# talmolab/sleap-nn

Measured on AMD Instinct MI355X. Metric: frames/sec bottom-up UNet 1024x1024 inference, higher is better.
Workload: dtype f32

## Files before the change

### sleap_nn_amd/csrc/w16_kernels.hip

```cpp
#include <type_traits>

#include "common.h"
#include "net_kernels.h"

namespace ph {

typedef float f32x4 __attribute__((ext_vector_type(4)));

constexpr int V_TW = 16, V_TH = 32;
constexpr int V_HH = V_TH + 2;
constexpr int V_PLANE_E = V_HH * 9;
constexpr int V_PLANE_PIECES = (V_PLANE_E + 15) / 16;
constexpr int V_PLANE_FLOATS = V_PLANE_PIECES * 256;
constexpr int V_HALO_FLOATS = 2 * V_PLANE_FLOATS;
constexpr int v_w_floats(int nb) { return 16 * nb * 256; }

__global__ __launch_bounds__(256) void w16_pack_kernel(const float* __restrict__ src, float* __restrict__ dst, int chunks, int nbs) {
  const int per = v_w_floats(nbs), total = chunks * per;
  for (int i = blockIdx.x * 256 + threadIdx.x; i < total; i += gridDim.x * 256) {
    const int chunk = i / per, r = i - chunk * per;
    const int e = r & 3, n = (r >> 2) & 15, kq = (r >> 6) & 3, nb = (r >> 8) % nbs, pos = (r >> 8) / nbs;
    const int xi = pos >> 2, nu = pos & 3;
    const int row = nb * 16 + n, kc = 4 * kq + e;
    const float* w = src + ((size_t)chunk * 9 * 32 + row) * 16 + kc;
    const int ts = 32 * 16;
    float h[3];
#pragma unroll
    for (int kx = 0; kx < 3; ++kx) {
      const float g0 = w[(0 * 3 + kx) * ts], g1 = w[(1 * 3 + kx) * ts], g2 = w[(2 * 3 + kx) * ts];
      h[kx] = xi == 0 ? g0 : (xi == 1 ? 0.5f * ((g0 + g2) + g1) : (xi == 2 ? 0.5f * ((g0 + g2) - g1) : g2));
    }
    dst[i] = nu == 0 ? h[0] : (nu == 1 ? 0.5f * ((h[0] + h[2]) + h[1]) : (nu == 2 ? 0.5f * ((h[0] + h[2]) - h[1]) : h[2]));
  }
}
int64_t w16_pack_floats(int chunks, int nbs) { return (int64_t)chunks * v_w_floats(nbs); }
int launch_w16_pack(const float* wpack, float* w16, int chunks, int nbs, hipStream_t s) {
  PH_REQUIRE(nbs == 1 || nbs == 2, "w16 pack: one or two N blocks of 16 channels");
  hipLaunchKernelGGL(w16_pack_kernel, dim3(std::min(chunks * v_w_floats(nbs) / 256, 256)), dim3(256), 0, s, wpack, w16, chunks, nbs);
  PH_HIP_CHECK(hipGetLastError());
  return PH_OK;
}

template <int CHUNKS, int NB, bool TWO = false, bool HEAD = false>
__global__ __launch_bounds__(512, 2) void conv3x3_w16_kernel(ConvArgs a) {
  constexpr int V_W_FLOATS = v_w_floats(NB);
  extern __shared__ __attribute__((aligned(16))) float lds[];
  float* const wl = lds;
  float* const hbuf = lds + CHUNKS * V_W_FLOATS;
  const int tid = threadIdx.x;
  const int lane = tid & 63;
  const int wave = __builtin_amdgcn_readfirstlane(tid >> 6);
  const int li = lane & 15, kq = lane >> 4;
  float m1 = -1.f;
  asm volatile("" : "+v"(m1));
  const int tiles_x = (a.W + V_TW - 1) / V_TW;
  const int tiles_y = (a.H + V_TH - 1) / V_TH;
  const int total = tiles_x * tiles_y * a.B;

  const __amdgpu_buffer_rsrc_t rsrc = __builtin_amdgcn_make_buffer_rsrc((void*)a.src0, 0, (int)((unsigned)(a.B * a.H * a.W) * (unsigned)(a.c0p * 4)), 0x00020000);
  const __amdgpu_buffer_rsrc_t rsrc1 = __builtin_amdgcn_make_buffer_rsrc((void*)(TWO ? a.src1 : a.src0), 0, (int)((unsigned)(a.B * a.H * a.W) * (unsigned)((TWO ? a.c1p : a.c0p) * 4)), 0x00020000);
  const int chunks0 = TWO ? a.c0p / 16 : CHUNKS;
  int hyx[5];
#pragma unroll
  for (int s = 0; s < 5; ++s) {
    const int p = wave + 8 * s;
    const int par = p >= V_PLANE_PIECES ? 1 : 0;
    const int e = (p - par * V_PLANE_PIECES) * 16 + (lane >> 2);
    const int hy = e / 9, hx = 2 * (e - hy * 9) + par;
    hyx[s] = e < V_PLANE_E ? (hy << 8) | hx : -1;
  }
  unsigned fvo[5], fvo1[5];
  auto tile_of = [&](int vid) { return (total & 7) == 0 ? (vid & 7) * (total >> 3) + (vid >> 3) : vid; };
  auto point = [&](int vid) {
    int t = tile_of(vid);
    const int tx = t % tiles_x;
    t /= tiles_x;
    const int ty = t % tiles_y;
    const int b = t / tiles_y;
    const int x0 = tx * V_TW, y0 = ty * V_TH;
    const unsigned base = (unsigned)((b * a.H + y0) * a.W + x0) * (unsigned)(a.c0p * 4);
#pragma unroll
    for (int s = 0; s < 5; ++s) {
      const int hy = hyx[s] >> 8, hx = hyx[s] & 255;
      const int gy = y0 + hy - 1, gx = x0 + hx - 1;
      const bool in = hyx[s] >= 0 && gy >= 0 && gy < a.H && gx >= 0 && gx < a.W;
      fvo[s] = in ? base + (unsigned)(((hy - 1) * a.W + (hx - 1)) * a.c0p * 4 + (lane & 3) * 16) : 0xFFFFFF00u;
      if (TWO) fvo1[s] = in ? (unsigned)(((b * a.H + gy) * a.W + gx) * a.c1p * 4 + (lane & 3) * 16) : 0xFFFFFF00u;
    }
  };
  auto dma = [&](float* buf, int chunk) {
    if (TWO && chunk >= chunks0) {
#pragma unroll
      for (int s = 0; s < 5; ++s)
        __builtin_amdgcn_raw_ptr_buffer_load_lds(rsrc1, (__attribute__((address_space(3))) void*)(buf + (wave + 8 * s) * 256), 16, fvo1[s], (chunk - chunks0) * 64, 0, 0);
      return;
    }
#pragma unroll
    for (int s = 0; s < 5; ++s)
      __builtin_amdgcn_raw_ptr_buffer_load_lds(rsrc, (__attribute__((address_space(3))) void*)(buf + (wave + 8 * s) * 256), 16, fvo[s], chunk * 64, 0, 0);
  };

  const int lbase = ((4 * wave + 2 * (li >> 3)) * 9 + (li & 7)) * 16 + kq * 4;
  auto a_off = [&](int r, int c) { return lbase + r * 9 * 16 + (c >> 1) * 16 + (c & 1) * V_PLANE_FLOATS; };
  const int boff = lane * 4;

  {
    const __amdgpu_buffer_rsrc_t wr = __builtin_amdgcn_make_buffer_rsrc((void*)a.wpack_w16, 0, CHUNKS * V_W_FLOATS * 4, 0x00020000);
    constexpr int WP = CHUNKS * 2 * NB;
#pragma unroll
    for (int s = 0; s < WP; ++s)
      __builtin_amdgcn_raw_ptr_buffer_load_lds(wr, (__attribute__((address_space(3))) void*)(wl + (wave * WP + s) * 256), 16, (unsigned)lane * 16u, (wave * WP + s) * 1024, 0, 0);
  }
  f32x4 hw[HEAD ? NB : 1];
  if (HEAD) {
#pragma unroll
    for (int nb = 0; nb < NB; ++nb) {
      hw[nb] = f32x4{0.f, 0.f, 0.f, 0.f};
      if (li < a.head_cout) hw[nb] = *reinterpret_cast<const f32x4*>(a.head_w + (size_t)li * a.head_wcp + nb * 16 + 4 * kq);
    }
  }
  int vid = blockIdx.x;
  point(vid);
  dma(hbuf, 0);
  __syncthreads();
  int par = 0;
  while (true) {
    const int nvid = vid + gridDim.x;
    const bool has_next = nvid < total;
    f32x4 acc[16][NB];
    if constexpr (CHUNKS > 1) {
#pragma unroll
      for (int p = 0; p < 16; ++p)
#pragma unroll
        for (int nb = 0; nb < NB; ++nb)
#pragma unroll
          for (int e = 0; e < 4; ++e) acc[p][nb][e] = 0.f;
    }
#pragma unroll 1
    for (int ch = 0; ch < CHUNKS; ++ch) {
      if (ch + 1 < CHUNKS) {
        dma(hbuf + (par ^ 1) * V_HALO_FLOATS, ch + 1);
      } else if (has_next) {
        point(nvid);
        dma(hbuf + (par ^ 1) * V_HALO_FLOATS, 0);
      }
      const float* hb = hbuf + par * V_HALO_FLOATS;
      const float* wc = wl + ch * V_W_FLOATS + boff;
      f32x4 da[4], db[4], av[4], bf[2][NB];
      auto read_rows = [&](int xi) {
        const int ra = xi == 0 ? 0 : (xi == 2 ? 2 : 1), rb = xi == 0 ? 2 : (xi == 1 ? 2 : (xi == 2 ? 1 : 3));
#pragma unroll
        for (int c = 0; c < 4; ++c) {
          da[c] = *reinterpret_cast<const f32x4*>(hb + a_off(ra, c));
          db[c] = *reinterpret_cast<const f32x4*>(hb + a_off(rb, c));
        }
      };
      auto load_b = [&](int pos, int fb) {
#pragma unroll
        for (int nb = 0; nb < NB; ++nb) bf[fb][nb] = *reinterpret_cast<const f32x4*>(wc + (pos * NB + nb) * 256);
      };
      read_rows(0);
      load_b(0, 0);
#pragma unroll
      for (int xi = 0; xi < 4; ++xi) {
        f32x4 t[4];
#pragma unroll
        for (int c = 0; c < 4; ++c) t[c] = xi == 1 ? da[c] + db[c] : db[c] * m1 + da[c];
        av[0] = t[2] * m1 + t[0];
        av[1] = t[1] + t[2];
        av[2] = t[1] * m1 + t[2];
        av[3] = t[3] * m1 + t[1];
#pragma unroll
        for (int c = 0; c < 4; ++c) asm volatile("" : "+v"(av[c]));
#pragma unroll
        for (int nu = 0; nu < 4; ++nu) {
          const int pos = xi * 4 + nu, cur = pos & 1;
#pragma unroll
          for (int nb = 0; nb < NB; ++nb)
            acc[pos][nb] = __builtin_amdgcn_mfma_f32_16x16x4f32(bf[cur][nb][0], av[nu][0], CHUNKS > 1 ? acc[pos][nb] : f32x4{0.f, 0.f, 0.f, 0.f}, 0, 0, 0);
          __builtin_amdgcn_sched_barrier(0);
          if (pos + 1 < 16) load_b(pos + 1, cur ^ 1);
          if (nu == 0 && xi + 1 < 4) read_rows(xi + 1);
          __builtin_amdgcn_sched_barrier(0);
#pragma unroll
          for (int j = 1; j < 4; ++j)
#pragma unroll
            for (int nb = 0; nb < NB; ++nb) acc[pos][nb] = __builtin_amdgcn_mfma_f32_16x16x4f32(bf[cur][nb][j], av[nu][j], acc[pos][nb], 0, 0, 0);
          __builtin_amdgcn_sched_barrier(0);
        }
      }
      __syncthreads();
      par ^= 1;
    }
    {
      int t = tile_of(vid);
      const int tx = t % tiles_x;
      t /= tiles_x;
      const int ty = t % tiles_y;
      const int b = t / tiles_y;
      const int x0 = tx * V_TW, y0 = ty * V_TH + 4 * wave;
      const bool interior = (x0 + V_TW <= a.W) && (y0 + 4 <= a.H);
      const int Hp = (a.H + 1) >> 1, Wp = (a.W + 1) >> 1;
      const int oy = y0 + 2 * (li >> 3), ox = x0 + 2 * (li & 7);
      f32x4 hd[2][2];
      if (HEAD) {
#pragma unroll
        for (int aa = 0; aa < 2; ++aa)
#pragma unroll
          for (int bb = 0; bb < 2; ++bb) hd[aa][bb] = f32x4{0.f, 0.f, 0.f, 0.f};
      }
#pragma unroll
      for (int nb = 0; nb < NB; ++nb) {
        const int co = nb * 16 + 4 * kq;
        const f32x4 bias = *reinterpret_cast<const f32x4*>(a.bias + co);
        f32x4 y[2][2];
        {
          f32x4 P[4][2];
#pragma unroll
          for (int xi = 0; xi < 4; ++xi) {
            P[xi][0] = (acc[xi * 4 + 0][nb] + acc[xi * 4 + 1][nb]) + acc[xi * 4 + 2][nb];
            P[xi][1] = acc[xi * 4 + 3][nb] * m1 + (acc[xi * 4 + 2][nb] * m1 + acc[xi * 4 + 1][nb]);
          }
#pragma unroll
          for (int bb = 0; bb < 2; ++bb) {
            const f32x4 v0 = ((P[0][bb] + P[1][bb]) + P[2][bb]) + bias, v1 = (P[3][bb] * m1 + (P[2][bb] * m1 + P[1][bb])) + bias;
#pragma unroll
            for (int e = 0; e < 4; ++e) {
              y[0][bb][e] = a.relu ? fmaxf(v0[e], 0.f) : v0[e];
              y[1][bb][e] = a.relu ? fmaxf(v1[e], 0.f) : v1[e];
            }
          }
        }
        if (HEAD) {
#pragma unroll
          for (int aa = 0; aa < 2; ++aa)
#pragma unroll
            for (int bb = 0; bb < 2; ++bb)
#pragma unroll
              for (int e = 0; e < 4; ++e) hd[aa][bb] = __builtin_amdgcn_mfma_f32_16x16x4f32(hw[nb][e], y[aa][bb][e], hd[aa][bb], 0, 0, 0);
        }
        if (!a.skip_dst) {
#pragma unroll
          for (int aa = 0; aa < 2; ++aa)
#pragma unroll
            for (int bb = 0; bb < 2; ++bb)
              if (interior || (oy + aa < a.H && ox + bb < a.W)) {
                const size_t o = ((size_t)(b * a.H + oy + aa) * a.W + ox + bb) * a.coutp + co;
                f32x4 v = y[aa][bb];
                if (a.relu_mask_src) {
                  const f32x4 f = *reinterpret_cast<const f32x4*>(a.relu_mask_src + o);
#pragma unroll
                  for (int e = 0; e < 4; ++e) v[e] = f[e] > 0.f ? v[e] : 0.f;
                }
                *reinterpret_cast<f32x4*>(a.dst + o) = v;
              }
        }
        if (a.dst_pool) {
          f32x4 pm;
#pragma unroll
          for (int e = 0; e < 4; ++e) {
            float v00 = y[0][0][e], v01 = y[0][1][e], v10 = y[1][0][e], v11 = y[1][1][e];
            if (!interior) {
              v00 = (oy < a.H && ox < a.W) ? v00 : 0.f;
              v01 = (oy < a.H && ox + 1 < a.W) ? v01 : 0.f;
              v10 = (oy + 1 < a.H && ox < a.W) ? v10 : 0.f;
              v11 = (oy + 1 < a.H && ox + 1 < a.W) ? v11 : 0.f;
            }
            pm[e] = fmaxf(fmaxf(v00, v01), fmaxf(v10, v11));
          }
          const int py = oy >> 1, px = ox >> 1;
          if (interior || (py < Hp && px < Wp)) *reinterpret_cast<f32x4*>(a.dst_pool + ((size_t)(b * Hp + py) * Wp + px) * a.coutp + co) = pm;
        }
      }
      if (HEAD) {
        const bool pair_ok = (a.W & 1) == 0;
#pragma unroll
        for (int r = 0; r < 4; ++r) {
          const int o = 4 * kq + r;
          if (o < a.head_cout) {
            const float hb = a.head_b[o];
#pragma unroll
            for (int aa = 0; aa < 2; ++aa) {
              if (oy + aa >= a.H || ox >= a.W) continue;
              float v0 = hd[aa][0][r] + hb, v1 = hd[aa][1][r] + hb;
              if (a.head_sigmoid) {
                v0 = 1.f / (1.f + expf(-v0));
                v1 = 1.f / (1.f + expf(-v1));
              }
              float* const hp = a.head_dst + (((size_t)b * a.head_cout + o) * a.H + oy + aa) * a.W + ox;
              const bool two = ox + 1 < a.W;
              if (two && pair_ok) {
                typedef float f32x2_t __attribute__((ext_vector_type(2)));
                f32x2_t v;
                v[0] = v0;
                v[1] = v1;
                *reinterpret_cast<f32x2_t*>(hp) = v;
              } else {
                hp[0] = v0;
                if (two) hp[1] = v1;
              }
            }
          }
        }
      }
    }
    if (!has_next) break;
    vid = nvid;
  }
}

static int v_cu_count(int* out) { return device_cu_count(out); }

int prepare_w16_kernels() {
  const void* ks[10] = {reinterpret_cast<const void*>(conv3x3_w16_kernel<1, 1, false, true>), reinterpret_cast<const void*>(conv3x3_w16_kernel<2, 2, false, true>),
                        reinterpret_cast<const void*>(conv3x3_w16_kernel<1, 1>), reinterpret_cast<const void*>(conv3x3_w16_kernel<2, 1>),
                       reinterpret_cast<const void*>(conv3x3_w16_kernel<1, 2>), reinterpret_cast<const void*>(conv3x3_w16_kernel<2, 2>),
                       reinterpret_cast<const void*>(conv3x3_w16_kernel<2, 1, true>), reinterpret_cast<const void*>(conv3x3_w16_kernel<3, 1, true>),
                       reinterpret_cast<const void*>(conv3x3_w16_kernel<4, 1, true>), reinterpret_cast<const void*>(conv3x3_w16_kernel<2, 2, true>)};
  for (const void* k : ks) {
    const hipError_t e = hipFuncSetAttribute(k, hipFuncAttributeMaxDynamicSharedMemorySize, 160 * 1024);
    if (e != hipSuccess) {
      set_error("hipFuncSetAttribute(w16) failed: %s", hipGetErrorString(e));
      return PH_E_HIP;
    }
  }
  return PH_OK;
}

bool w16_shape_ok(int c0p, int c1p, int coutp) {
  if (coutp != 16 && coutp != 32) return false;
  const int chunks = (c0p + c1p) / 16;
  if (c1p == 0) return c0p == 16 || c0p == 32;
  return (c0p % 16) == 0 && (c1p % 16) == 0 && c0p > 0 && chunks >= 2 && chunks <= (coutp == 16 ? 4 : 2);
}
bool w16_fits(const ConvArgs& a) {
  const uint64_t px = (uint64_t)a.B * a.H * a.W;
  return a.wpack_w16 && a.bn == 32 && w16_shape_ok(a.c0p, a.src1 ? a.c1p : 0, a.coutp) && (a.src1 != nullptr) == (a.c1p > 0) && !a.src1_lowres && !a.accumulate &&
         px * (uint64_t)a.c0p * 4 < 0xFFFFFF00ull && px * (uint64_t)a.c1p * 4 < 0xFFFFFF00ull && px < 0x7FFFFFFFull;
}

bool w16_takes_head(const ConvArgs& a) {
  return w16_fits(a) && !a.src1 && !a.dst_pool && !a.relu_mask_src && ((a.c0p == 16 && a.coutp == 16) || (a.c0p == 32 && a.coutp == 32));
}

int launch_conv3x3_w16(const ConvArgs& a, hipStream_t s) {
  PH_REQUIRE(w16_fits(a), "w16: Cout 16 or 32 (one N tile), 16 or 32 input channels from one source or 2 - 4 chunks from two, no accumulate, sources below 4 GiB");
  int n_cu = 0;
  const int rc = v_cu_count(&n_cu);
  if (rc != PH_OK) return rc;
  const int tiles = ((a.W + V_TW - 1) / V_TW) * ((a.H + V_TH - 1) / V_TH) * a.B;
  const int chunks = (a.c0p + a.c1p) / 16, nbs = a.coutp / 16;
  const size_t ldsb = (size_t)(chunks * v_w_floats(nbs) + 2 * V_HALO_FLOATS) * sizeof(float);
  const dim3 grid(std::min(tiles, n_cu));
  if (a.head_w) {
    PH_REQUIRE(w16_takes_head(a) && a.head_cout >= 1 && a.head_cout <= 16 && a.head_wcp == a.coutp && a.head_b && a.head_dst, "w16: a fused head needs 16 -> 16 or 32 -> 32 channels from one source, no pool, and at most 16 head channels");
    if (nbs == 1)
      hipLaunchKernelGGL((conv3x3_w16_kernel<1, 1, false, true>), grid, dim3(512), ldsb, s, a);
    else
      hipLaunchKernelGGL((conv3x3_w16_kernel<2, 2, false, true>), grid, dim3(512), ldsb, s, a);
  } else if (a.src1 && nbs == 2)
    hipLaunchKernelGGL((conv3x3_w16_kernel<2, 2, true>), grid, dim3(512), ldsb, s, a);
  else if (a.src1 && chunks == 2)
    hipLaunchKernelGGL((conv3x3_w16_kernel<2, 1, true>), grid, dim3(512), ldsb, s, a);
  else if (a.src1 && chunks == 3)
    hipLaunchKernelGGL((conv3x3_w16_kernel<3, 1, true>), grid, dim3(512), ldsb, s, a);
  else if (a.src1)
    hipLaunchKernelGGL((conv3x3_w16_kernel<4, 1, true>), grid, dim3(512), ldsb, s, a);
  else if (chunks == 1 && nbs == 1)
    hipLaunchKernelGGL((conv3x3_w16_kernel<1, 1>), grid, dim3(512), ldsb, s, a);
  else if (chunks == 2 && nbs == 1)
    hipLaunchKernelGGL((conv3x3_w16_kernel<2, 1>), grid, dim3(512), ldsb, s, a);
  else if (chunks == 1)
    hipLaunchKernelGGL((conv3x3_w16_kernel<1, 2>), grid, dim3(512), ldsb, s, a);
  else
    hipLaunchKernelGGL((conv3x3_w16_kernel<2, 2>), grid, dim3(512), ldsb, s, a);
  PH_HIP_CHECK(hipGetLastError());
  return PH_OK;
}

}
```

Before: 3088.

## Restructure w16 conv kernel: peel first chunk, fast interior addressing, batched epilogue

Peels the first input-channel chunk so accumulators start from zero in the MFMA instead of explicit zeroing. Precomputes relative halo offsets so interior tiles skip per-element bounds checks. Rewrites the epilogue to compute all output blocks before storing, using the compile-time channel stride and bitmask-based masking for pooling. It also adds experiment macros and a clock probe, disabled by default, which makes the change partly a probing scaffold and may shift register pressure.

```diff
diff --git a/sleap_nn_amd/csrc/w16_kernels.hip b/sleap_nn_amd/csrc/w16_kernels.hip
--- a/sleap_nn_amd/csrc/w16_kernels.hip
+++ b/sleap_nn_amd/csrc/w16_kernels.hip
@@ -2,6 +2,10 @@
 
 #include "common.h"
 #include "net_kernels.h"
+
+#ifndef W16_EXP
+#define W16_EXP 0
+#endif
 
 namespace ph {
 
@@ -14,6 +18,15 @@
 constexpr int V_PLANE_FLOATS = V_PLANE_PIECES * 256;
 constexpr int V_HALO_FLOATS = 2 * V_PLANE_FLOATS;
 constexpr int v_w_floats(int nb) { return 16 * nb * 256; }
+
+__device__ __forceinline__ f32x4 w16_mfma(float wgt, float x, f32x4 c) {
+#if W16_EXP & 4
+  asm volatile("" ::"v"(wgt), "v"(x));
+  return c;
+#else
+  return __builtin_amdgcn_mfma_f32_16x16x4f32(wgt, x, c, 0, 0, 0);
+#endif
+}
 
 __global__ __launch_bounds__(256) void w16_pack_kernel(const float* __restrict__ src, float* __restrict__ dst, int chunks, int nbs) {
   const int per = v_w_floats(nbs), total = chunks * per;
@@ -44,6 +57,7 @@
 template <int CHUNKS, int NB, bool TWO = false, bool HEAD = false>
 __global__ __launch_bounds__(512, 2) void conv3x3_w16_kernel(ConvArgs a) {
   constexpr int V_W_FLOATS = v_w_floats(NB);
+  constexpr int COUTP = 16 * NB;
   extern __shared__ __attribute__((aligned(16))) float lds[];
   float* const wl = lds;
   float* const hbuf = lds + CHUNKS * V_W_FLOATS;
@@ -56,11 +70,15 @@
   const int tiles_x = (a.W + V_TW - 1) / V_TW;
   const int tiles_y = (a.H + V_TH - 1) / V_TH;
   const int total = tiles_x * tiles_y * a.B;
+#ifdef W16_CLOCK
+  const unsigned long long clk_c0 = __builtin_amdgcn_s_memtime(), clk_r0 = __builtin_amdgcn_s_memrealtime();
+#endif
 
   const __amdgpu_buffer_rsrc_t rsrc = __builtin_amdgcn_make_buffer_rsrc((void*)a.src0, 0, (int)((unsigned)(a.B * a.H * a.W) * (unsigned)(a.c0p * 4)), 0x00020000);
   const __amdgpu_buffer_rsrc_t rsrc1 = __builtin_amdgcn_make_buffer_rsrc((void*)(TWO ? a.src1 : a.src0), 0, (int)((unsigned)(a.B * a.H * a.W) * (unsigned)((TWO ? a.c1p : a.c0p) * 4)), 0x00020000);
   const int chunks0 = TWO ? a.c0p / 16 : CHUNKS;
   int hyx[5];
+  unsigned rel[5], rel1[5];
 #pragma unroll
   for (int s = 0; s < 5; ++s) {
     const int p = wave + 8 * s;
@@ -68,6 +86,8 @@
     const int e = (p - par * V_PLANE_PIECES) * 16 + (lane >> 2);
     const int hy = e / 9, hx = 2 * (e - hy * 9) + par;
     hyx[s] = e < V_PLANE_E ? (hy << 8) | hx : -1;
+    rel[s] = (unsigned)(((hy - 1) * a.W + (hx - 1)) * a.c0p * 4 + (lane & 3) * 16);
+    if (TWO) rel1[s] = (unsigned)(((hy - 1) * a.W + (hx - 1)) * a.c1p * 4 + (lane & 3) * 16);
   }
   unsigned fvo[5], fvo1[5];
   auto tile_of = [&](int vid) { return (total & 7) == 0 ? (vid & 7) * (total >> 3) + (vid >> 3) : vid; };
@@ -78,17 +98,28 @@
     const int ty = t % tiles_y;
     const int b = t / tiles_y;
     const int x0 = tx * V_TW, y0 = ty * V_TH;
-    const unsigned base = (unsigned)((b * a.H + y0) * a.W + x0) * (unsigned)(a.c0p * 4);
+    const unsigned pix = (unsigned)((b * a.H + y0) * a.W + x0);
+    const unsigned base = pix * (unsigned)(a.c0p * 4);
+    const unsigned base1 = TWO ? pix * (unsigned)(a.c1p * 4) : 0u;
+    if (x0 >= 1 && y0 >= 1 && x0 + V_TW + 1 <= a.W && y0 + V_TH + 1 <= a.H) {
+#pragma unroll
+      for (int s = 0; s < 5; ++s) {
+        fvo[s] = hyx[s] >= 0 ? base + rel[s] : 0xFFFFFF00u;
+        if (TWO) fvo1[s] = hyx[s] >= 0 ? base1 + rel1[s] : 0xFFFFFF00u;
+      }
+      return;
+    }
 #pragma unroll
     for (int s = 0; s < 5; ++s) {
       const int hy = hyx[s] >> 8, hx = hyx[s] & 255;
       const int gy = y0 + hy - 1, gx = x0 + hx - 1;
       const bool in = hyx[s] >= 0 && gy >= 0 && gy < a.H && gx >= 0 && gx < a.W;
-      fvo[s] = in ? base + (unsigned)(((hy - 1) * a.W + (hx - 1)) * a.c0p * 4 + (lane & 3) * 16) : 0xFFFFFF00u;
-      if (TWO) fvo1[s] = in ? (unsigned)(((b * a.H + gy) * a.W + gx) * a.c1p * 4 + (lane & 3) * 16) : 0xFFFFFF00u;
+      fvo[s] = in ? base + rel[s] : 0xFFFFFF00u;
+      if (TWO) fvo1[s] = in ? base1 + rel1[s] : 0xFFFFFF00u;
     }
   };
   auto dma = [&](float* buf, int chunk) {
+    if (W16_EXP & 1) return;
     if (TWO && chunk >= chunks0) {
 #pragma unroll
       for (int s = 0; s < 5; ++s)
@@ -101,7 +132,7 @@
   };
 
   const int lbase = ((4 * wave + 2 * (li >> 3)) * 9 + (li & 7)) * 16 + kq * 4;
-  auto a_off = [&](int r, int c) { return lbase + r * 9 * 16 + (c >> 1) * 16 + (c & 1) * V_PLANE_FLOATS; };
+  auto a_off = [&](int r, int c) { return r * 9 * 16 + (c >> 1) * 16 + (c & 1) * V_PLANE_FLOATS; };
   const int boff = lane * 4;
 
   {
@@ -128,23 +159,17 @@
     const int nvid = vid + gridDim.x;
     const bool has_next = nvid < total;
     f32x4 acc[16][NB];
-    if constexpr (CHUNKS > 1) {
-#pragma unroll
-      for (int p = 0; p < 16; ++p)
-#pragma unroll
-        for (int nb = 0; nb < NB; ++nb)
-#pragma unroll
-          for (int e = 0; e < 4; ++e) acc[p][nb][e] = 0.f;
-    }
-#pragma unroll 1
-    for (int ch = 0; ch < CHUNKS; ++ch) {
+    auto unit = [&](auto first_c, int ch) {
+      constexpr bool FIRST = decltype(first_c)::value;
       if (ch + 1 < CHUNKS) {
         dma(hbuf + (par ^ 1) * V_HALO_FLOATS, ch + 1);
       } else if (has_next) {
         point(nvid);
         dma(hbuf + (par ^ 1) * V_HALO_FLOATS, 0);
       }
-      const float* hb = hbuf + par * V_HALO_FLOATS;
+      int ho = CHUNKS * V_W_FLOATS + par * V_HALO_FLOATS + lbase;
+      asm volatile("" : "+v"(ho));
+      const float* hb = lds + ho;
       const float* wc = wl + ch * V_W_FLOATS + boff;
       f32x4 da[4], db[4], av[4], bf[2][NB];
       auto read_rows = [&](int xi) {
@@ -170,6 +195,10 @@
         av[1] = t[1] + t[2];
         av[2] = t[1] * m1 + t[2];
         av[3] = t[3] * m1 + t[1];
+        if (W16_EXP & 16) {
+#pragma unroll
+          for (int c = 0; c < 4; ++c) av[c] = xi & 1 ? da[c] : db[c];
+        }
 #pragma unroll
         for (int c = 0; c < 4; ++c) asm volatile("" : "+v"(av[c]));
 #pragma unroll
@@ -177,7 +206,7 @@
           const int pos = xi * 4 + nu, cur = pos & 1;
 #pragma unroll
           for (int nb = 0; nb < NB; ++nb)
-            acc[pos][nb] = __builtin_amdgcn_mfma_f32_16x16x4f32(bf[cur][nb][0], av[nu][0], CHUNKS > 1 ? acc[pos][nb] : f32x4{0.f, 0.f, 0.f, 0.f}, 0, 0, 0);
+            acc[pos][nb] = w16_mfma(bf[cur][nb][0], av[nu][0], FIRST ? f32x4{0.f, 0.f, 0.f, 0.f} : acc[pos][nb]);
           __builtin_amdgcn_sched_barrier(0);
           if (pos + 1 < 16) load_b(pos + 1, cur ^ 1);
           if (nu == 0 && xi + 1 < 4) read_rows(xi + 1);
@@ -185,13 +214,16 @@
 #pragma unroll
           for (int j = 1; j < 4; ++j)
 #pragma unroll
-            for (int nb = 0; nb < NB; ++nb) acc[pos][nb] = __builtin_amdgcn_mfma_f32_16x16x4f32(bf[cur][nb][j], av[nu][j], acc[pos][nb], 0, 0, 0);
+            for (int nb = 0; nb < NB; ++nb) acc[pos][nb] = w16_mfma(bf[cur][nb][j], av[nu][j], acc[pos][nb]);
           __builtin_amdgcn_sched_barrier(0);
         }
       }
-      __syncthreads();
+      if (!(W16_EXP & 8)) __syncthreads();
       par ^= 1;
-    }
+    };
+    unit(std::true_type{}, 0);
+#pragma unroll 1
+    for (int ch = 1; ch < CHUNKS; ++ch) unit(std::false_type{}, ch);
     {
       int t = tile_of(vid);
       const int tx = t % tiles_x;
@@ -202,74 +234,118 @@
       const bool interior = (x0 + V_TW <= a.W) && (y0 + 4 <= a.H);
       const int Hp = (a.H + 1) >> 1, Wp = (a.W + 1) >> 1;
       const int oy = y0 + 2 * (li >> 3), ox = x0 + 2 * (li & 7);
+      f32x4 y[NB][2][2];
+#pragma unroll
+      for (int nb = 0; nb < NB; ++nb) {
+        const f32x4 bias = *reinterpret_cast<const f32x4*>(a.bias + nb * 16 + 4 * kq);
+        f32x4 P[4][2];
+#pragma unroll
+        for (int xi = 0; xi < 4; ++xi) {
+          P[xi][0] = (acc[xi * 4 + 0][nb] + acc[xi * 4 + 1][nb]) + acc[xi * 4 + 2][nb];
+          P[xi][1] = acc[xi * 4 + 3][nb] * m1 + (acc[xi * 4 + 2][nb] * m1 + acc[xi * 4 + 1][nb]);
+        }
+#pragma unroll
+        for (int bb = 0; bb < 2; ++bb) {
+          y[nb][0][bb] = ((P[0][bb] + P[1][bb]) + P[2][bb]) + bias;
+          y[nb][1][bb] = (P[3][bb] * m1 + (P[2][bb] * m1 + P[1][bb])) + bias;
+        }
+      }
+      if (a.relu) {
+#pragma unroll
+        for (int nb = 0; nb < NB; ++nb)
+#pragma unroll
+          for (int aa = 0; aa < 2; ++aa)
+#pragma unroll
+            for (int bb = 0; bb < 2; ++bb)
+#pragma unroll
+              for (int e = 0; e < 4; ++e) y[nb][aa][bb][e] = fmaxf(y[nb][aa][bb][e], 0.f);
+      }
       f32x4 hd[2][2];
       if (HEAD) {
 #pragma unroll
         for (int aa = 0; aa < 2; ++aa)
 #pragma unroll
-          for (int bb = 0; bb < 2; ++bb) hd[aa][bb] = f32x4{0.f, 0.f, 0.f, 0.f};
-      }
-#pragma unroll
-      for (int nb = 0; nb < NB; ++nb) {
-        const int co = nb * 16 + 4 * kq;
-        const f32x4 bias = *reinterpret_cast<const f32x4*>(a.bias + co);
-        f32x4 y[2][2];
-        {
-          f32x4 P[4][2];
-#pragma unroll
-          for (int xi = 0; xi < 4; ++xi) {
-            P[xi][0] = (acc[xi * 4 + 0][nb] + acc[xi * 4 + 1][nb]) + acc[xi * 4 + 2][nb];
-            P[xi][1] = acc[xi * 4 + 3][nb] * m1 + (acc[xi * 4 + 2][nb] * m1 + acc[xi * 4 + 1][nb]);
+          for (int bb = 0; bb < 2; ++bb) {
+            hd[aa][bb] = f32x4{0.f, 0.f, 0.f, 0.f};
+#pragma unroll
+            for (int nb = 0; nb < NB; ++nb)
+#pragma unroll
+              for (int e = 0; e < 4; ++e) hd[aa][bb] = __builtin_amdgcn_mfma_f32_16x16x4f32(hw[nb][e], y[nb][aa][bb][e], hd[aa][bb], 0, 0, 0);
           }
-#pragma unroll
-          for (int bb = 0; bb < 2; ++bb) {
-            const f32x4 v0 = ((P[0][bb] + P[1][bb]) + P[2][bb]) + bias, v1 = (P[3][bb] * m1 + (P[2][bb] * m1 + P[1][bb])) + bias;
-#pragma unroll
-            for (int e = 0; e < 4; ++e) {
-              y[0][bb][e] = a.relu ? fmaxf(v0[e], 0.f) : v0[e];
-              y[1][bb][e] = a.relu ? fmaxf(v1[e], 0.f) : v1[e];
+      }
+      bool ok[2][2];
+#pragma unroll
+      for (int aa = 0; aa < 2; ++aa)
+#pragma unroll
+        for (int bb = 0; bb < 2; ++bb) ok[aa][bb] = interior || (oy + aa < a.H && ox + bb < a.W);
+      if (W16_EXP & 2) {
+#pragma unroll
+        for (int nb = 0; nb < NB; ++nb)
+#pragma unroll
+          for (int aa = 0; aa < 2; ++aa)
+#pragma unroll
+            for (int bb = 0; bb < 2; ++bb) asm volatile("" ::"v"(y[nb][aa][bb]));
+      }
+      if (!a.skip_dst && !(W16_EXP & 2)) {
+        const size_t o = ((size_t)(b * a.H + oy) * a.W + ox) * COUTP + 4 * kq;
+        const size_t row = (size_t)a.W * COUTP;
+        float* const dp = a.dst + o;
+        if (a.relu_mask_src) {
+          const float* const mp = a.relu_mask_src + o;
+#pragma unroll
+          for (int nb = 0; nb < NB; ++nb)
+#pragma unroll
+            for (int aa = 0; aa < 2; ++aa)
+#pragma unroll
+              for (int bb = 0; bb < 2; ++bb)
+                if (ok[aa][bb]) {
+                  const f32x4 f = *reinterpret_cast<const f32x4*>(mp + aa * row + bb * COUTP + nb * 16);
+                  f32x4 v = y[nb][aa][bb];
+#pragma unroll
+                  for (int e = 0; e < 4; ++e) v[e] = f[e] > 0.f ? v[e] : 0.f;
+                  *reinterpret_cast<f32x4*>(dp + aa * row + bb * COUTP + nb * 16) = v;
+                }
+        } else if (interior) {
+#pragma unroll
+          for (int nb = 0; nb < NB; ++nb)
+#pragma unroll
+            for (int aa = 0; aa < 2; ++aa)
+#pragma unroll
+              for (int bb = 0; bb < 2; ++bb) *reinterpret_cast<f32x4*>(dp + aa * row + bb * COUTP + nb * 16) = y[nb][aa][bb];
+        } else {
+#pragma unroll
+          for (int nb = 0; nb < NB; ++nb)
+#pragma unroll
+            for (int aa = 0; aa < 2; ++aa)
+#pragma unroll
+              for (int bb = 0; bb < 2; ++bb)
+                if (ok[aa][bb]) *reinterpret_cast<f32x4*>(dp + aa * row + bb * COUTP + nb * 16) = y[nb][aa][bb];
+        }
+      }
+      if (a.dst_pool && !(W16_EXP & 2)) {
+        if (!interior) {
+#pragma unroll
+          for (int aa = 0; aa < 2; ++aa)
+#pragma unroll
+            for (int bb = 0; bb < 2; ++bb) {
+              unsigned keep = ok[aa][bb] ? 0xFFFFFFFFu : 0u;
+              asm volatile("" : "+v"(keep));
+#pragma unroll
+              for (int nb = 0; nb < NB; ++nb)
+#pragma unroll
+                for (int e = 0; e < 4; ++e) y[nb][aa][bb][e] = __uint_as_float(__float_as_uint(y[nb][aa][bb][e]) & keep);
             }
+        }
+        const int py = oy >> 1, px = ox >> 1;
+        if (interior || (py < Hp && px < Wp)) {
+          float* const pp = a.dst_pool + ((size_t)(b * Hp + py) * Wp + px) * COUTP + 4 * kq;
+#pragma unroll
+          for (int nb = 0; nb < NB; ++nb) {
+            f32x4 pm;
+#pragma unroll
+            for (int e = 0; e < 4; ++e) pm[e] = fmaxf(fmaxf(y[nb][0][0][e], y[nb][0][1][e]), fmaxf(y[nb][1][0][e], y[nb][1][1][e]));
+            *reinterpret_cast<f32x4*>(pp + nb * 16) = pm;
           }
-        }
-        if (HEAD) {
-#pragma unroll
-          for (int aa = 0; aa < 2; ++aa)
-#pragma unroll
-            for (int bb = 0; bb < 2; ++bb)
-#pragma unroll
-              for (int e = 0; e < 4; ++e) hd[aa][bb] = __builtin_amdgcn_mfma_f32_16x16x4f32(hw[nb][e], y[aa][bb][e], hd[aa][bb], 0, 0, 0);
-        }
-        if (!a.skip_dst) {
-#pragma unroll
-          for (int aa = 0; aa < 2; ++aa)
-#pragma unroll
-            for (int bb = 0; bb < 2; ++bb)
-              if (interior || (oy + aa < a.H && ox + bb < a.W)) {
-                const size_t o = ((size_t)(b * a.H + oy + aa) * a.W + ox + bb) * a.coutp + co;
-                f32x4 v = y[aa][bb];
-                if (a.relu_mask_src) {
-                  const f32x4 f = *reinterpret_cast<const f32x4*>(a.relu_mask_src + o);
-#pragma unroll
-                  for (int e = 0; e < 4; ++e) v[e] = f[e] > 0.f ? v[e] : 0.f;
-                }
-                *reinterpret_cast<f32x4*>(a.dst + o) = v;
-              }
-        }
-        if (a.dst_pool) {
-          f32x4 pm;
-#pragma unroll
-          for (int e = 0; e < 4; ++e) {
-            float v00 = y[0][0][e], v01 = y[0][1][e], v10 = y[1][0][e], v11 = y[1][1][e];
-            if (!interior) {
-              v00 = (oy < a.H && ox < a.W) ? v00 : 0.f;
-              v01 = (oy < a.H && ox + 1 < a.W) ? v01 : 0.f;
-              v10 = (oy + 1 < a.H && ox < a.W) ? v10 : 0.f;
-              v11 = (oy + 1 < a.H && ox + 1 < a.W) ? v11 : 0.f;
-            }
-            pm[e] = fmaxf(fmaxf(v00, v01), fmaxf(v10, v11));
-          }
-          const int py = oy >> 1, px = ox >> 1;
-          if (interior || (py < Hp && px < Wp)) *reinterpret_cast<f32x4*>(a.dst_pool + ((size_t)(b * Hp + py) * Wp + px) * a.coutp + co) = pm;
         }
       }
       if (HEAD) {
@@ -307,6 +383,13 @@
     if (!has_next) break;
     vid = nvid;
   }
+#ifdef W16_CLOCK
+  __syncthreads();
+  if (a.clock_probe && tid == 0) {
+    a.clock_probe[blockIdx.x * 2] = __builtin_amdgcn_s_memtime() - clk_c0;
+    a.clock_probe[blockIdx.x * 2 + 1] = __builtin_amdgcn_s_memrealtime() - clk_r0;
+  }
+#endif
 }
 
 static int v_cu_count(int* out) { return device_cu_count(out); }
```

New measurement: 3105, median of 6. Within noise of the previous version (+0.6%).
